# dotchen/LearningByCheating

Hardware: AMD Instinct MI355X
Metric: images/sec ImagePolicyModelSS phase-1 train @ bs256 (higher is better)
Workload: dtype bf16; 1 GPU; ImagePolicyModelSS(resnet34) phase-1 step vs BirdViewPolicyModelSS(resnet18) teacher [phase1_bs256_bf16], 160x384 RGB + 7x192x192 bird-view uint8 NHWC frames as the dataset stores them (2048-frame dataset per rank resident in HBM, a different batch every step), global batch 256 (256/GPU), bf16 MFMA operands and bf16 activation storage + f32 accumulate/master weights/gradients/BN/loss/Adam, local B; global_batch=256, parallelism=dp1

## Files before the change

### learningbycheating_amd/csrc/engine.cpp

```cpp
#include "engine.hpp"

#include <algorithm>
#include <stdlib.h>
#include <string.h>

namespace lbc {

namespace {
constexpr float kBnMomentum = 0.1f;
constexpr float kBnEps = 1e-5f;
size_t up64(size_t n) { return (n + 63) / 64 * 64; }
#define LBC_TRY(expr)            \
    do {                         \
        int rc__ = (expr);       \
        if (rc__) return rc__;   \
    } while (0)
}

int Net::add_tensor(const std::string& name, int kind, std::initializer_list<int> shape)
{
    TensorInfo ti;
    ti.name = name;
    ti.kind = kind;
    ti.ndim = (int)shape.size();
// ... 339 lines not shown
    if (!fn) { sync_fn_ = nullptr; sync_ctx_ = nullptr; sync_world_ = 1; sync_buf_ = nullptr; return LBC_OK; }
    LBC_REQUIRE(world >= 1 && buf && buf_floats >= kSyncFloats, "net.set_sync_bn: world_size >= 1 and a buffer of >= %d floats",
                kSyncFloats);
    sync_fn_ = fn; sync_ctx_ = ctx; sync_world_ = world; sync_buf_ = buf;
    return LBC_OK;
}

int Net::sync_rows(const float*& part, int& rows, int width, int n_local, hipStream_t s, float* local_lo, float* local_hi)
{
    if (!sync_fn_) return LBC_OK;
    LBC_REQUIRE(width + 1 <= kSyncFloats, "net: %d sums do not fit the SyncBN buffer", width);
    if (rows > kLbcFinalizeRows) {
        LBC_TRY(lbc_partial_reduce(part, rows, width, W(partial2_), 64, s));
        part = W(partial2_); rows = 64;
    }
    LBC_TRY(lbc_partial_reduce(part, rows, width, sync_buf_, 1, s, local_lo, local_hi, (float)n_local));
    if (sync_fn_(sync_ctx_, sync_buf_, width + 1, s) != 0) {
        lbc_set_error("net: the SyncBN all-reduce callback failed");
        return LBC_ELAUNCH;
    }
    part = sync_buf_; rows = 1;
    return LBC_OK;
}

int Net::bn_finalize(const BN& bn, int rows, long long count, int n_local, int train, hipStream_t s, bool update_running, const float* synced)
{
    const float* part = W(partial_);
    const float* nsum = nullptr;
    if (train && synced) {
        part = synced; rows = 1; nsum = synced + 2 * bn.C;
    } else if (train && sync_fn_) {
        LBC_TRY(sync_rows(part, rows, 2 * bn.C, n_local, s));
        nsum = part + 2 * bn.C;
    } else if (train && rows > kLbcFinalizeRows) {
        LBC_TRY(lbc_partial_reduce(W(partial_), rows, 2 * bn.C, W(partial2_), 64, s));
        part = W(partial2_);
        rows = 64;
    }
    BnFinalizeArgs f = fin_args(bn, part, rows, count, update_running);
    f.nsum = nsum; f.n_local = n_local; f.train = train;
    if (!train) { f.running_mean = P(bn.rm); f.running_var = P(bn.rv); f.num_batches_tracked = nullptr; }
    return lbc_bn_finalize(f, s);
}

BnFinalizeArgs Net::fin_args(const BN& bn, const float* part, int rows, long long count, bool update_running) const
{
    BnFinalizeArgs f;
    memset(&f, 0, sizeof(f));
    f.partial = part; f.rows = rows; f.C = bn.C; f.count = count;
    f.gamma = P(bn.g); f.beta = P(bn.b);
    f.running_mean = update_running ? P(bn.rm) : nullptr;
    f.running_var = update_running ? P(bn.rv) : nullptr;
    f.num_batches_tracked = update_running ? static_cast<long long*>(t_[bn.nbt].ptr) : nullptr;
    f.momentum = kBnMomentum; f.eps = kBnEps; f.train = 1;
    f.scale = W(bn.scale); f.shift = W(bn.shift); f.save_mean = W(bn.mean); f.save_invstd = W(bn.invstd);
    return f;
}

int Net::forward(int N, int train, const void* image, int image_u8, const float* velocity, const float* command, float* pred_sel,
                 float* pred_all, hipStream_t s)
{
    LBC_REQUIRE(N >= 1 && N <= d_.max_batch, "net.forward: batch %d outside [1,%d]", N, d_.max_batch);
    LBC_REQUIRE(image && velocity && command && pred_all, "net.forward: null argument");
    LBC_TRY(check_bound(false));
    lastN_ = N; last_train_ = train; ++generation_;
    const int H0 = d_.H, W0 = d_.W, Cin = d_.in_channels;
    const bool tr = train != 0;
    int rows = 0;

    LBC_TRY(lbc_copy_f32(command, W(cmd_), 4 * N, s));
    NormConst nc;
    memset(&nc, 0, sizeof(nc));
    nc.enabled = d_.normalize;
    const float m3[3] = {0.485f, 0.456f, 0.406f}, s3[3] = {0.229f, 0.224f, 0.225f};
    for (int i = 0; i < 3; ++i) { nc.mean[i] = m3[i]; nc.stdv[i] = s3[i]; }
    if (image_u8) LBC_TRY(lbc_prep_input_u8(static_cast<const unsigned char*>(image), W(xp_), bf16_, N, Cin, H0, W0, nc, s));
    else          LBC_TRY(lbc_prep_input(static_cast<const float*>(image), W(xp_), bf16_, N, Cin, H0, W0, nc, s));
    const bool reuse = frozen_ && derived_valid_ && !tr;
    if (act_bf16_ && !reuse) LBC_TRY(weight_prep(s));
    if (!tr && !reuse) LBC_TRY(bn_eval_prep(s));
    derived_valid_ = frozen_ && !tr;

    StemArgs st;
    st.xp = W(xp_); st.xp_bf16 = bf16_; st.w = P(stem_w_); st.y = W(y0_); st.stats = tr ? W(partial_) : nullptr;
    st.N = N; st.H = H0; st.W = W0; st.Cin = Cin; st.act_bf16 = act_bf16_; st.bf16 = bf16_;
    LBC_TRY(lbc_stem_fwd(st, s));
    if (tr) LBC_TRY(bn_finalize(stem_bn_, lbc_stem_rows(st), (long long)N * (H0 / 2) * (W0 / 2), N, train, s));
    PoolFwdArgs pf;
    pf.y = W(y0_); pf.scale = W(stem_bn_.scale); pf.shift = W(stem_bn_.shift); pf.p = W(p0_);
    pf.idx = reinterpret_cast<unsigned char*>(W(idx_));
    pf.N = N; pf.H = H0 / 2; pf.W = W0 / 2; pf.C = 64; pf.act_bf16 = act_bf16_;
    LBC_TRY(lbc_bn_relu_maxpool_fwd(pf, s));

    const float* x = W(p0_);
    for (Block& b : blocks_) {
        const long long pix = (long long)N * b.c1.OH * b.c1.OW;
        if (!tr) {
            LBC_TRY(conv_fwd(b.c1, x, N, false, &rows, s, nullptr, &b.b1, nullptr, true));
            const float* identity = x;
            if (b.has_ds) {
                LBC_TRY(conv_fwd(b.ds, x, N, false, &rows, s, nullptr, &b.bd, nullptr, false));
                identity = W(b.ds.y);
            }
            LBC_TRY(conv_fwd(b.c2, W(b.c1.y), N, false, &rows, s, nullptr, &b.b2, identity, true, W(b.out)));
            x = W(b.out);
            continue;
        }
        LBC_TRY(conv_fwd(b.c1, x, N, tr, &rows, s));
        const bool fold1 = !b.fuse_z1 && can_fold(rows, b.b1.C);
        if (!fold1) LBC_TRY(bn_finalize(b.b1, rows, pix, N, train, s));
        BnApplyArgs ap;
        if (b.fuse_z1) {
            LBC_TRY(conv_fwd(b.c2, W(b.c1.y), N, tr, &rows, s, &b.b1));
        } else {
            memset(&ap, 0, sizeof(ap));
            ap.x = W(b.c1.y); ap.y = W(b.z1); ap.pixels = pix; ap.C = b.c1.Cout;
            ap.scale = W(b.b1.scale); ap.shift = W(b.b1.shift); ap.relu = 1; ap.act_bf16 = act_bf16_;
            if (fold1) { ap.fold = 1; ap.fin = fin_args(b.b1, W(partial_), rows, pix); }
            LBC_TRY(lbc_bn_apply(ap, s));
            LBC_TRY(conv_fwd(b.c2, W(b.z1), N, tr, &rows, s));
        }
        const bool fold2 = can_fold(rows, b.b2.C) && (!b.has_ds || (size_t)lbc_cdiv(pix, 64) * 2 * b.bd.C <= partial2_floats_);
        const int rows2 = rows;
        if (!fold2) LBC_TRY(bn_finalize(b.b2, rows, pix, N, train, s));
        memset(&ap, 0, sizeof(ap));
        ap.x = W(b.c2.y); ap.y = W(b.out); ap.pixels = pix; ap.C = b.c2.Cout;
        ap.scale = W(b.b2.scale); ap.shift = W(b.b2.shift); ap.relu = 1; ap.act_bf16 = act_bf16_;
        if (fold2) { ap.fold = 1; ap.fin = fin_args(b.b2, W(partial_), rows2, pix); }
        if (b.has_ds) {
            float* dsp = fold2 ? W(partial2_) : W(partial_);
            LBC_TRY(conv_fwd(b.ds, x, N, tr, &rows, s, nullptr, nullptr, nullptr, false, nullptr, dsp, fold2 ? partial2_floats_ : partial_floats_));
            if (fold2 && can_fold(rows, b.bd.C)) { ap.rfold = 1; ap.rfin = fin_args(b.bd, dsp, rows, pix); }
            else if (fold2) LBC_TRY(lbc_bn_finalize(fin_args(b.bd, dsp, rows, pix), s));
            else LBC_TRY(bn_finalize(b.bd, rows, pix, N, train, s));
            ap.resid = W(b.ds.y); ap.rscale = W(b.bd.scale); ap.rshift = W(b.bd.shift);
        } else {
            ap.resid = x;
        }
        LBC_TRY(lbc_bn_apply(ap, s));
        x = W(b.out);
    }

    const Block& last = blocks_.back();
    const int th = last.c2.OH, tw = last.c2.OW;
    LBC_TRY(lbc_concat_velocity(x, velocity, W(hcat_), N, th * tw, 512, 128, act_bf16_, s));
    if (tr) {
        ChanReduceArgs cr;
        memset(&cr, 0, sizeof(cr));
        cr.x = W(hcat_); cr.partial = W(partial_); cr.pixels = (long long)N * th * tw; cr.C = 640; cr.act_bf16 = act_bf16_;
        cr.max_rows = fold_rows_for(cr.pixels, 640);
        LBC_TRY(lbc_chan_reduce(cr, 0, s));
        rows = lbc_chan_reduce_rows(cr.pixels, 640, cr.max_rows);
    }
    int pend_rows = rows;
    long long pend_count = (long long)N * th * tw;
    const float* din = W(hcat_);
    for (int i = 0; i < 3; ++i) {
        Deconv& D = dec_[i];
        IgemmArgs a;
        memset(&a, 0, sizeof(a));
        a.x = din; a.w = P(D.w); a.y = W(D.u); a.bias = P(D.bias); a.relu = 1;
        a.pre_scale = W(D.bn.scale); a.pre_shift = W(D.bn.shift);
        a.N = N; a.H = D.H; a.W = D.W; a.C = D.Cin;
        a.OH = 2 * D.H; a.OW = 2 * D.W; a.K = D.Cout;
        a.KH = 3; a.KW = 3; a.S = 2; a.P = 1;
        a.LH = D.H; a.LW = D.W; a.ostep = 2;
        a.M = N * D.H * D.W;
        a.stats = tr ? W(partial_) : nullptr;
        a.act_bf16 = act_bf16_;
        int wmajor = 0;
        if (act_bf16_) {
            a.w = W(D.wt); a.w_bf16 = 1; a.bf16 = 1; wmajor = 1;
        } else if (bf16_) {
            LBC_TRY(lbc_weight_transpose(P(D.w), W(wt_), D.Cin, 9, D.Cout, s));
            a.w = W(wt_); a.bf16 = 1; wmajor = 1;
// ... 624 lines not shown
```

### learningbycheating_amd/csrc/lbc_common.hpp

```cpp
#pragma once
#include <hip/hip_runtime.h>
#include <stddef.h>
#include <stdint.h>

typedef float f32x4 __attribute__((ext_vector_type(4)));
typedef float f32x16 __attribute__((ext_vector_type(16)));

#define LBC_OK 0
#define LBC_EINVAL (-1)
#define LBC_ELAUNCH (-2)
#define LBC_ESTATE (-3)

void lbc_set_error(const char* fmt, ...);
int lbc_check_launch(const char* what);

#define LBC_REQUIRE(cond, ...)                 \
    do {                                       \
        if (!(cond)) {                         \
            lbc_set_error(__VA_ARGS__);        \
            return LBC_EINVAL;                 \
        }                                      \
    } while (0)

static inline int lbc_cdiv(long long a, long long b) { return (int)((a + b - 1) / b); }

enum LbcOpt {
    kOptForceCfg = 0,
    kOptHaloBlocks,
    kOptHeadNoMfma,
    kOptNoSideStream,
    kOptNoGemm256,
    kOptGemm256MinTiles,
    kOptGemm256Cfg,
    kOptNoBnBwdFuse,
    kOptNoHdma,
    kOptHdmaCfg,
    kOptNoGldsPhased,
    kOptHdmaPersistWgs,
    kOptWgradTr2MinWgs,
    kOptNoC64pPre,
    kOptNoBnFold,
    kOptC64pBm,
    kOptHdmapSplit,
    kOptHdmaSmallBelow,
    kOptCount
};
long long lbc_opt(LbcOpt o);
static inline bool lbc_opt_on(LbcOpt o) { return lbc_opt(o) == 1; }

bool lbc_prof_on();
void lbc_prof_begin(const char* name, double flops, double bytes, hipStream_t s);
void lbc_prof_end(hipStream_t s);
void lbc_prof_note(const char* name, double bytes);
struct LbcProfScope {
    hipStream_t s; bool on;
    LbcProfScope(const char* name, double flops, double bytes, hipStream_t st) : s(st), on(lbc_prof_on()) {
        if (on) lbc_prof_begin(name, flops, bytes, s);
    }
    ~LbcProfScope() { if (on) lbc_prof_end(s); }
};

struct IgemmArgs {
    const void* x;
    const void* w;
    void* y;
    const float* post_scale;
    const float* post_shift;
    const float* bias;
    const void* resid;
    float* stats;
    const float* pre_scale;
    const float* pre_shift;
    int pre_relu;
    int N, H, W, C;
    int OH, OW, K;
    int KH, KW, S, P;
    int M;
    int LH, LW;
    int oy0, ox0, ostep;
    int nphase;
    int relu;
    int stat_row0;
    int bf16;
    int act_bf16;
    int w_bf16;
    const void* bnb_y;
    const float* bnb_scale;
    const float* bnb_shift;
    const float* bnb_mean;
    const float* bnb_invstd;
    const void* bnb_mask;
    float* split_ws;
    long long split_ws_floats;
};
bool lbc_igemm_fuses_bn_bwd(const IgemmArgs& a, int wmajor, int mode, int cfg);
bool lbc_igemm_fuses_bn_bwd_masked(const IgemmArgs& a, int wmajor, int mode, int cfg);

struct WeightPrepItem {
    const float* w;
    void* wn;
    void* wt;
    int A, T, B;
    int tile_begin;
};
static inline int lbc_weight_prep_tiles(int A, int T, int B) { return lbc_cdiv(A, 64) * lbc_cdiv(B, 64) * T; }
struct WeightPrepArgs {
    static const int kMax = 48;
    WeightPrepItem item[kMax];
    int count;
    int tiles;
};
int lbc_weight_prep(const WeightPrepArgs& a, hipStream_t s);

int lbc_igemm_rows(const IgemmArgs& a, int cfg);
int lbc_igemm_pick(long long M, int K);
int lbc_igemm_pick_for(const IgemmArgs& a, int mode);
constexpr int kLbcCfgGlds = 3;
constexpr int kLbcGldsCfgs = 7;
constexpr int kLbcCfgHdma = kLbcCfgGlds + kLbcGldsCfgs;
constexpr int kLbcHdmaCfgs = 5;
int lbc_conv_hdma_pick(const IgemmArgs& a, int mode);
int lbc_conv_hdma_rows(const IgemmArgs& a, int cfg);
int lbc_conv_hdma_launch(const IgemmArgs& a, int mode, int cfg, hipStream_t s);
int lbc_conv_c64p_launch(const IgemmArgs& a, int mode, hipStream_t s);
int lbc_conv_c64p_rows(const IgemmArgs& a);
bool lbc_conv_hdmap_phased(const IgemmArgs& a, int mode);
bool lbc_conv_hdmap_eligible(const IgemmArgs& a, int mode, int cfg);
// ... 50 lines not shown
```

### learningbycheating_amd/csrc/lbc_kernels.hpp

```cpp
#pragma once
#include "lbc_common.hpp"

constexpr int kLbcFinalizeRows = 1024;
struct BnFinalizeArgs {
    const float* partial;
    int rows, C;
    long long count;
    const float* nsum; int n_local;
    const float* gamma;
    const float* beta;
    float* running_mean;
    float* running_var;
    long long* num_batches_tracked;
    float* more_running_mean[3]; float* more_running_var[3]; long long* more_num_batches_tracked[3];
    float momentum, eps;
    int train;
    float* scale;
    float* shift;
    float* save_mean;
    float* save_invstd;
};
struct BnEvalItem {
    const float* gamma; const float* beta; const float* running_mean; const float* running_var;
    float* scale; float* shift; float* mean; float* invstd;
// ... 2 lines not shown
struct BnEvalArgs {
    static const int kMax = 48;
    BnEvalItem item[kMax];
    int count;
    float eps;
};
int lbc_bn_eval_prep(const BnEvalArgs& a, hipStream_t s);
int lbc_partial_reduce(const float* in, int rows, int cols, float* out, int out_rows, hipStream_t s, float* copy_lo = nullptr,
                       float* copy_hi = nullptr, float tail = -1.f);
int lbc_bn_finalize(const BnFinalizeArgs& a, hipStream_t s);

struct BnApplyArgs {
    const void* x; void* y;
    long long pixels; int C;
    const float* scale; const float* shift;
    const void* resid;
    const float* rscale;
    const float* rshift;
    int relu;
    int act_bf16;
    int fold, rfold;
    BnFinalizeArgs fin, rfin;
};
int lbc_bn_apply(const BnApplyArgs& a, hipStream_t s);
bool lbc_bn_fold_ok(int rows, int C);
int lbc_bn_fold_max_rows(int C);

struct ChanReduceArgs {
    const void* x;
    const void* dz;
    const void* mask;
    const float* mask_scale;
    const float* mask_shift;
    void* g_out;
    const float* mean;
    const float* invstd;
    float* partial;
    long long pixels; int C;
    long long pix_per_block;
    int act_bf16;
    int max_rows;
};
int lbc_chan_reduce_rows(long long pixels, int C, int max_rows = 0);
int lbc_chan_reduce(ChanReduceArgs a, int op, hipStream_t s);

struct BnBwdFinalizeArgs {
    const float* partial; int rows, C; long long count;
    const float* nsum; int n_local;
    const float* gamma; const float* mean; const float* invstd;
    int train;
    float* dgamma; float* dbeta;
    float* coefA; float* coefB; float* coefD;
};
int lbc_bn_bwd_finalize(const BnBwdFinalizeArgs& a, hipStream_t s);

struct BnBwdApplyArgs {
    const void* g; const void* mask; const void* x;
    const float* coefA; const float* coefB; const float* coefD;
    const float* mean; const float* invstd;
    void* dx;
    long long pixels; int C, Cout;
    int accum;
    int act_bf16;
    int fold;
    BnBwdFinalizeArgs fin;
};
int lbc_bn_bwd_apply(const BnBwdApplyArgs& a, hipStream_t s);

int lbc_copy_f32(const float* src, float* dst, long long n, hipStream_t s);
int lbc_concat_velocity(const void* t, const float* vel, void* h, int N, int hw, int Ct, int Cv, int act_bf16, hipStream_t s);

struct NormConst { float mean[8]; float stdv[8]; int enabled; };
int lbc_prep_input(const float* img_nchw, void* xp, int xp_bf16, int N, int C, int H, int W, const NormConst& nc, hipStream_t s);
int lbc_prep_input_u8(const unsigned char* img_nhwc, void* xp, int xp_bf16, int N, int C, int H, int W, const NormConst& nc, hipStream_t s);
struct StemArgs {
    const void* xp;
    int xp_bf16;
    const float* w;
    void* y;
    float* stats;
    int N, H, W, Cin;
    int act_bf16;
    int bf16;
};
int lbc_stem_rows(const StemArgs& a);
int lbc_stem_fwd(const StemArgs& a, hipStream_t s);
struct StemWgradArgs {
    const void* xp; int xp_bf16; const void* dy; float* partial;
    int N, H, W, Cin, nsplit;
    int act_bf16;
    int bf16;
    const void* bn_y;
    const float* bn_coefA; const float* bn_coefB; const float* bn_coefD; const float* bn_mean; const float* bn_invstd;
};
bool lbc_stem_wgrad_fuses_bn_bwd(int Cin, int bf16);
int lbc_stem_wgrad_split(int N, int H, int W, int Cin, int bf16);
int lbc_stem_wgrad(const StemWgradArgs& a, hipStream_t s);

struct PoolFwdArgs {
    const void* y;
    const float* scale; const float* shift;
    void* p;
    unsigned char* idx;
    int N, H, W, C;
    int act_bf16;
};
int lbc_bn_relu_maxpool_fwd(const PoolFwdArgs& a, hipStream_t s);
struct PoolBwdArgs {
    const void* dp;
    const unsigned char* idx;
    const void* y;
    const float* scale; const float* shift;
    const float* mean; const float* invstd;
    void* g;
    float* partial;
    int N, H, W, C;
    long long pix_per_block;
    int act_bf16;
};
int lbc_pool_bwd_rows(int N, int H, int W, int C);
int lbc_maxpool_relu_bwd_reduce(PoolBwdArgs a, hipStream_t s);

struct HeadArgs {
    const void* h;
    int act_bf16;
    const float* mean[4];
    const float* invstd[4];
    const float* gamma[4];
    const float* beta[4];
    const float* w[4];
    const float* bias[4];
    const float* cmd;
    const float* pos_x[4];
    const float* pos_y[4];
    float* pred_all;
    float* pred_sel;
    float* rowstat;
    int N, OH, OW;
    float* scratch;
    int nslice;
    int wsplit;
};
int lbc_head_fwd(const HeadArgs& a, hipStream_t s);
struct HeadBwdArgs {
    HeadArgs f;
    const float* d_all;
    const float* d_sel;
    float* s_partial;
    void* dh;
    const float* chan_coef;
};
int lbc_head_bwd_rows(const HeadArgs& f);
int lbc_head_bwd_max_rows(int max_batch);
int lbc_head_bwd_reduce(const HeadBwdArgs& a, hipStream_t s);
struct HeadBwdFinalizeArgs {
    const float* s_partial; int rows; long long count;
    const float* nsum; int n_local;
    const float* gamma[4]; const float* beta[4]; const float* w[4];
    const float* mean; const float* invstd;
    float* dgamma[4]; float* dbeta[4]; float* dw[4]; float* dbias[4];
    float* chan_coef;
    int coef_only;
};
int lbc_head_bwd_finalize(const HeadBwdFinalizeArgs& a, hipStream_t s);
int lbc_head_bwd_apply(const HeadBwdArgs& a, hipStream_t s);

enum { kAugBlur = 0, kAugNoise = 1, kAugCoarseDropout = 2, kAugDropout = 3, kAugAdd = 4, kAugMultiply = 5, kAugContrast = 6 };
struct WarpParams {
    double im[6];
// ... 35 lines not shown
```

### learningbycheating_amd/csrc/lbc_util.cpp

```cpp
#include "lbc_common.hpp"
#include <stdarg.h>
#include <stdio.h>

static thread_local char g_err[512] = "";

void lbc_set_error(const char* fmt, ...)
{
    va_list ap;
    va_start(ap, fmt);
    vsnprintf(g_err, sizeof(g_err), fmt, ap);
    va_end(ap);
}

int lbc_check_launch(const char* what)
{
    hipError_t e = hipGetLastError();
    if (e != hipSuccess) {
        lbc_set_error("%s: launch failed: %s", what, hipGetErrorString(e));
        return LBC_ELAUNCH;
    }
    return LBC_OK;
}

extern "C" const char* lbc_last_error(void) { return g_err; }

#include <stdlib.h>
#include <mutex>
extern "C" char** environ;
#include <string.h>
namespace {
const char* const kOptNames[kOptCount] = {
    "LBC_FORCE_CFG", "LBC_HALO_BLOCKS", "LBC_HEAD_NO_MFMA", "LBC_NO_SIDE_STREAM", "LBC_NO_GEMM256", "LBC_GEMM256_MIN_TILES", "LBC_GEMM256_CFG",
    "LBC_NO_BN_BWD_FUSE", "LBC_NO_HDMA", "LBC_HDMA_CFG", "LBC_NO_GLDS_PHASED", "LBC_HDMA_PERSIST_WGS", "LBC_WGRAD_TR2_MIN_WGS", "LBC_NO_C64P_PRE",
    "LBC_NO_BN_FOLD", "LBC_C64P_BM", "LBC_HDMAP_SPLIT", "LBC_HDMA_SMALL_BELOW"};
struct OptTable {
    long long v[kOptCount];
    OptTable()
    {
        for (int i = 0; i < kOptCount; ++i) {
            const char* e = getenv(kOptNames[i]);
            v[i] = (e && *e) ? atoll(e) : -1;
        }
        for (char** ep = environ; ep && *ep; ++ep) {
            if (strncmp(*ep, "LBC_", 4)) continue;
            const char* eq = strchr(*ep, '=');
            const size_t n = eq ? (size_t)(eq - *ep) : strlen(*ep);
            bool known = (n == 17 && !strncmp(*ep, "LBC_PROF_LAUNCHES", n)) || (n == 15 && !strncmp(*ep, "LBC_PIN_STAGING", n)) || !strncmp(*ep, "LBC_ARCH", 8) || !strncmp(*ep, "LBC_BUILD_", 10) || !strncmp(*ep, "LBC_TEST_", 9) || !strncmp(*ep, "LBC_EMU_", 8);
            for (int i = 0; i < kOptCount && !known; ++i) known = strlen(kOptNames[i]) == n && !strncmp(*ep, kOptNames[i], n);
            if (!known) fprintf(stderr, "liblbc_hip: environment variable %.*s is not an option of this library (ignored); see include/lbc_hip.h, lbc_config_set\n", (int)n, *ep);
        }
    }
};
OptTable& opts() { static OptTable t; return t; }
}
long long lbc_opt(LbcOpt o) { return opts().v[o]; }
extern "C" int lbc_config_set(const char* name, long long value)
{
    LBC_REQUIRE(name, "config_set: null name");
    for (int i = 0; i < kOptCount; ++i)
        if (!strcmp(name, kOptNames[i])) { opts().v[i] = value; return LBC_OK; }
    lbc_set_error("config_set: unknown option %s", name);
    return LBC_EINVAL;
}
extern "C" long long lbc_config_get(const char* name)
{
    if (name)
        for (int i = 0; i < kOptCount; ++i)
            if (!strcmp(name, kOptNames[i])) return opts().v[i];
    return -1;
}

int lbc_zero_page(const void** p)
{
    static void* pages[64] = {nullptr};
    static std::mutex mu;
    int dev = 0;
    if (hipGetDevice(&dev) != hipSuccess || dev < 0 || dev >= 64) { lbc_set_error("zero_page: bad device"); return LBC_ELAUNCH; }
    std::lock_guard<std::mutex> lock(mu);
    if (!pages[dev]) {
        void* q = nullptr;
        if (hipMalloc(&q, 256) != hipSuccess || hipMemset(q, 0, 256) != hipSuccess) { lbc_set_error("zero_page: allocation failed"); return LBC_ELAUNCH; }
        pages[dev] = q;
    }
    *p = pages[dev];
    return LBC_OK;
}

#include <map>
#include <string>
#include <vector>
namespace {
struct ProfRec { const char* name; double flops, bytes; hipEvent_t e0, e1; };
bool g_prof = false;
std::vector<ProfRec> g_recs;
}
bool lbc_prof_on() { return g_prof; }
void lbc_prof_begin(const char* name, double flops, double bytes, hipStream_t s)
{
    ProfRec r;
    r.name = name; r.flops = flops; r.bytes = bytes;
    (void)hipEventCreate(&r.e0); (void)hipEventCreate(&r.e1);
    (void)hipEventRecord(r.e0, s);
    g_recs.push_back(r);
}
void lbc_prof_end(hipStream_t s) { if (!g_recs.empty()) (void)hipEventRecord(g_recs.back().e1, s); }
void lbc_prof_note(const char* name, double bytes)
{
    ProfRec r;
    r.name = name; r.flops = 0.0; r.bytes = bytes; r.e0 = nullptr; r.e1 = nullptr;
    if (g_recs.empty()) g_recs.push_back(r); else g_recs.insert(g_recs.end() - 1, r);
}

extern "C" int lbc_profile_enable(int on)
{
    g_prof = on != 0;
    return 0;
}
// ... 31 lines not shown
```

### learningbycheating_amd/csrc/stem.hip

```cpp
#include "lbc_common.hpp"
#include "lbc_act.hpp"
#include "lbc_kernels.hpp"
#include <type_traits>

namespace {

template <typename XT>
__global__ __launch_bounds__(256) void prep_input_k(const float* __restrict__ img, XT* __restrict__ xp, int N, int C,
                                                    int H, int W, NormConst nc)
{
    const int Hp = H + 6, Wp = W + 6;
    const long long total = (long long)N * Hp * Wp;
    const long long stride = (long long)gridDim.x * blockDim.x;
    for (long long i = (long long)blockIdx.x * blockDim.x + threadIdx.x; i < total; i += stride) {
        const int xq = (int)(i % Wp);
        const long long t = i / Wp;
        const int yq = (int)(t % Hp);
        const int n = (int)(t / Hp);
        const int x = xq - 3, y = yq - 3;
        const bool in = (unsigned)x < (unsigned)W && (unsigned)y < (unsigned)H;
        XT* dst = xp + (size_t)i * C;
        for (int c = 0; c < C; ++c) {
            float v = 0.f;
            if (in) {
// ... 625 lines not shown
        for (int q = 0; q < NLD; ++q)
            if (br[q] < 7) *reinterpret_cast<unsigned*>(&sBand[buf][br[q] * RS + bj[q] * 4]) = regs[q];
    };

    float s1 = 0.f, s2 = 0.f;
    int tile, tend, it = 0;
    {
        const int nwg = gridDim.x, b = blockIdx.x;
        const int xcd = b & 7, q = nwg >> 3, rr = nwg & 7;
        const int logical = (xcd < rr ? xcd * (q + 1) : rr * (q + 1) + (xcd - rr) * q) + (b >> 3);
        const int per = (ntiles + nwg - 1) / nwg;
        tile = logical * per;
        tend = tile + per < ntiles ? tile + per : ntiles;
    }
    if (tile < tend) band_load(tile);
    __syncthreads();
    if (tile < tend) band_store(0);
    __syncthreads();
    for (; tile < tend; ++tile, ++it) {
        const int buf = it & 1;
        const int next = tile + 1 < tend ? tile + 1 : ntiles;
        if (next < ntiles) band_load(next);
        const int xt = tile % tiles_x;
        const int t2 = tile / tiles_x;
        const int oy = t2 % OH, n = t2 / OH;
        const int ox0 = xt * BX;
        f32x16 acc;
#pragma unroll
        for (int e = 0; e < 16; ++e) acc[e] = 0.f;
        const char* band = &sBand[buf][0] + ((32 * wm + l31) * 2 * CIN + 8 * kh) * 2;
#pragma unroll
        for (int r = 0; r < 7; ++r)
#pragma unroll
            for (int g = 0; g < KG; ++g) {
                const unsigned* src = reinterpret_cast<const unsigned*>(band + r * RS + g * 32);
                typedef unsigned u32x4 __attribute__((ext_vector_type(4)));
                const u32x4 raw = {src[0], src[1], src[2], src[3]};
                acc = __builtin_amdgcn_mfma_f32_32x32x16_bf16(__builtin_bit_cast(bf16x8, raw), bw[r][g], acc, 0, 0, 0);
            }
        const int col = 32 * wn + l31;
#pragma unroll
        for (int e = 0; e < 16; ++e) {
            const int prow = 32 * wm + (e & 3) + 8 * (e >> 2) + 4 * kh;
            const float v = acc[e];
            Act<T>::st1(&sOut[prow * OLD + col], v);
            if (ox0 + prow < OW) { s1 += v; s2 += v * v; }
        }
        if (next < ntiles) band_store(buf ^ 1);
        __syncthreads();
        {
            constexpr int EPT = 16;
            const int prow = tid >> 2, c0 = (tid & 3) * EPT;
            if (ox0 + prow < OW) {
                T* dst = static_cast<T*>(a.y) + ((size_t)(n * OH + oy) * OW + (size_t)(ox0 + prow)) * 64 + c0;
                const T* srcp = &sOut[prow * OLD + c0];
#pragma unroll
                for (int v = 0; v < EPT * (int)sizeof(T) / 16; ++v)
                    reinterpret_cast<f32x4*>(dst)[v] = reinterpret_cast<const f32x4*>(srcp)[v];
            }
        }
        __syncthreads();
    }
    if (a.stats) {
        s1 += __shfl_xor(s1, 32);
        s2 += __shfl_xor(s2, 32);
        if (kh == 0) { sRed[wm][0][32 * wn + l31] = s1; sRed[wm][1][32 * wn + l31] = s2; }
        __syncthreads();
        if (tid < 64) {
            float* dst = a.stats + (size_t)blockIdx.x * 2 * 64;
            dst[tid] = sRed[0][0][tid] + sRed[1][0][tid];
            dst[64 + tid] = sRed[0][1][tid] + sRed[1][1][tid];
        }
    }
}

static int stem_rows_grid(int N, int H, int W, int Cin)
{
    const long long tiles = (long long)N * (H / 2) * lbc_cdiv(W / 2, 64);
    const long long grid = 256 * (Cin == 3 ? 3 : 2);
    return (int)(tiles < grid ? tiles : grid);
}
static bool stem_fwd_rows(const StemArgs& a) { return a.bf16 != 0; }

}

int lbc_prep_input_u8(const unsigned char* img_nhwc, void* xp, int xp_bf16, int N, int C, int H, int W, const NormConst& nc, hipStream_t s)
{
    LBC_REQUIRE(C <= 8, "prep_input: at most 8 channels");
    const long long total = (long long)N * (H + 6) * (W + 6);
    long long blocks = (total + 255) / 256;
    if (blocks > 4096) blocks = 4096;
    LbcProfScope prof("prep_input", 0.0, 1.0 * N * H * (double)W * C + (xp_bf16 ? 2.0 : 4.0) * (double)total * C, s);
    const bool small = total + blocks * 256 < (1ll << 31);
#define LBC_PU(XT, CINv)                                                                                                                 \
    do {                                                                                                                                 \
        if (small) hipLaunchKernelGGL((prep_input_u8_k<XT, CINv, unsigned>), dim3((unsigned)blocks), dim3(256), 0, s, img_nhwc, static_cast<XT*>(xp), N, C, H, W, nc);  \
        else       hipLaunchKernelGGL((prep_input_u8_k<XT, CINv, long long>), dim3((unsigned)blocks), dim3(256), 0, s, img_nhwc, static_cast<XT*>(xp), N, C, H, W, nc); \
    } while (0)
#define LBC_PUC(XT)                                                                                                                      \
    do {                                                                                                                                 \
        if (C == 3) LBC_PU(XT, 3);                                                                                                       \
        else if (C == 7) LBC_PU(XT, 7);                                                                                                  \
        else LBC_PU(XT, 0);                                                                                                              \
    } while (0)
    if (xp_bf16) LBC_PUC(__bf16);
    else         LBC_PUC(float);
#undef LBC_PUC
#undef LBC_PU
    return lbc_check_launch("prep_input_u8");
}

int lbc_prep_input(const float* img_nchw, void* xp, int xp_bf16, int N, int C, int H, int W, const NormConst& nc, hipStream_t s)
{
    LBC_REQUIRE(C <= 8, "prep_input: at most 8 channels");
    const long long total = (long long)N * (H + 6) * (W + 6);
    long long blocks = (total + 255) / 256;
    if (blocks > 4096) blocks = 4096;
    LbcProfScope prof("prep_input", 0.0, 4.0 * N * H * (double)W * C + (xp_bf16 ? 2.0 : 4.0) * (double)total * C, s);
    if (xp_bf16) hipLaunchKernelGGL(prep_input_k<__bf16>, dim3((unsigned)blocks), dim3(256), 0, s, img_nchw, static_cast<__bf16*>(xp), N, C, H, W, nc);
    else         hipLaunchKernelGGL(prep_input_k<float>, dim3((unsigned)blocks), dim3(256), 0, s, img_nchw, static_cast<float*>(xp), N, C, H, W, nc);
    return lbc_check_launch("prep_input");
}

int lbc_stem_rows(const StemArgs& a)
{
    if (stem_fwd_rows(a)) return stem_rows_grid(a.N, a.H, a.W, a.Cin);
    return lbc_cdiv((long long)a.N * (a.H / 2) * (a.W / 2), 128);
}

int lbc_stem_fwd(const StemArgs& a, hipStream_t s)
{
    LBC_REQUIRE(a.Cin == 3 || a.Cin == 7, "stem: Cin=%d unsupported (3 or 7)", a.Cin);
    LBC_REQUIRE(a.H % 2 == 0 && a.W % 2 == 0, "stem: odd image size");
    LBC_REQUIRE((long long)a.N * (a.H + 6) * (a.W + 6) * a.Cin < (1ll << 31), "stem: input too large");
    const dim3 grid((unsigned)lbc_stem_rows(a));
    const double Ms = (double)a.N * (a.H / 2) * (a.W / 2);
    LbcProfScope prof("stem_fwd", 2.0 * Ms * 64 * 49 * a.Cin, (a.xp_bf16 ? 2.0 : 4.0) * (double)a.N * (a.H + 6) * (a.W + 6) * a.Cin + (a.act_bf16 ? 2.0 : 4.0) * Ms * 64, s);
    LBC_REQUIRE(!a.act_bf16 || a.bf16, "stem: bf16 output needs bf16 = 1");
    if (stem_fwd_rows(a)) {
        LBC_REQUIRE(a.xp_bf16, "stem: the bf16 kernels read a bf16 padded image");
        const int tx = lbc_cdiv(a.W / 2, 64);
        const int ntiles = a.N * (a.H / 2) * tx;
#define LBC_K(T, CI) hipLaunchKernelGGL((stem_fwd_rows_k<CI, T>), grid, dim3(256), 0, s, a, ntiles, tx)
        if (a.Cin == 3) LBC_DISPATCH_ACT(a.act_bf16, LBC_K, 3);
        else            LBC_DISPATCH_ACT(a.act_bf16, LBC_K, 7);
#undef LBC_K
        return lbc_check_launch("stem_fwd");
    }
    if (a.Cin == 3) hipLaunchKernelGGL((stem_fwd_k<3, float>), grid, dim3(256), 0, s, a);
    else            hipLaunchKernelGGL((stem_fwd_k<7, float>), grid, dim3(256), 0, s, a);
    return lbc_check_launch("stem_fwd");
}

static bool stem_wgrad_rows(int Cin, int bf16) { return bf16 && Cin == 3; }
bool lbc_stem_wgrad_fuses_bn_bwd(int Cin, int bf16) { return stem_wgrad_rows(Cin, bf16) && !lbc_opt_on(kOptNoBnBwdFuse); }

int lbc_stem_wgrad_split(int N, int H, int W, int Cin, int bf16)
{
    if (stem_wgrad_rows(Cin, bf16)) {
        const long long chunks = ((long long)N * (H / 2) * (W / 2) + 63) / 64;
        long long ng = chunks / 8;
        if (ng > 512) ng = 512;
        if (ng < 1) ng = 1;
        return (int)(2 * ng);
    }
    const long long chunks = ((long long)N * (H / 2) * (W / 2) + 31) / 32;
// ... 42 lines not shown
```

Baseline: 18150 images/sec.

## Fuse eval-mode stem conv with BN, ReLU and maxpool into one kernel

Adds a kernel that computes the 7x7 stride-2 stem convolution with MFMA, then applies the 3x3/2 maxpool and the folded BN scale/shift plus ReLU in the same pass. It uses the sign of gamma so the max can be taken before the affine step. It is used only in eval-mode forward, i.e. the frozen teacher, and removes the full-resolution stem activation round trip through HBM and the separate pool kernel. In exchange it adds a complex row-band pipeline with overlap recompute across work-unit boundaries and shared-memory carry state.

```diff
diff --git a/learningbycheating_amd/csrc/engine.cpp b/learningbycheating_amd/csrc/engine.cpp
--- a/learningbycheating_amd/csrc/engine.cpp
+++ b/learningbycheating_amd/csrc/engine.cpp
@@ -445,15 +445,21 @@
     derived_valid_ = frozen_ && !tr;
 
     StemArgs st;
+    memset(&st, 0, sizeof(st));
     st.xp = W(xp_); st.xp_bf16 = bf16_; st.w = P(stem_w_); st.y = W(y0_); st.stats = tr ? W(partial_) : nullptr;
     st.N = N; st.H = H0; st.W = W0; st.Cin = Cin; st.act_bf16 = act_bf16_; st.bf16 = bf16_;
-    LBC_TRY(lbc_stem_fwd(st, s));
-    if (tr) LBC_TRY(bn_finalize(stem_bn_, lbc_stem_rows(st), (long long)N * (H0 / 2) * (W0 / 2), N, train, s));
-    PoolFwdArgs pf;
-    pf.y = W(y0_); pf.scale = W(stem_bn_.scale); pf.shift = W(stem_bn_.shift); pf.p = W(p0_);
-    pf.idx = reinterpret_cast<unsigned char*>(W(idx_));
-    pf.N = N; pf.H = H0 / 2; pf.W = W0 / 2; pf.C = 64; pf.act_bf16 = act_bf16_;
-    LBC_TRY(lbc_bn_relu_maxpool_fwd(pf, s));
+    if (!tr && lbc_stem_pool_ok(H0, W0, Cin, act_bf16_, bf16_)) {
+        st.y = nullptr; st.gamma = P(stem_bn_.g); st.scale = W(stem_bn_.scale); st.shift = W(stem_bn_.shift); st.p = W(p0_);
+        LBC_TRY(lbc_stem_pool_fwd(st, s));
+    } else {
+        LBC_TRY(lbc_stem_fwd(st, s));
+        if (tr) LBC_TRY(bn_finalize(stem_bn_, lbc_stem_rows(st), (long long)N * (H0 / 2) * (W0 / 2), N, train, s));
+        PoolFwdArgs pf;
+        pf.y = W(y0_); pf.scale = W(stem_bn_.scale); pf.shift = W(stem_bn_.shift); pf.p = W(p0_);
+        pf.idx = reinterpret_cast<unsigned char*>(W(idx_));
+        pf.N = N; pf.H = H0 / 2; pf.W = W0 / 2; pf.C = 64; pf.act_bf16 = act_bf16_;
+        LBC_TRY(lbc_bn_relu_maxpool_fwd(pf, s));
+    }
 
     const float* x = W(p0_);
     for (Block& b : blocks_) {
diff --git a/learningbycheating_amd/csrc/lbc_common.hpp b/learningbycheating_amd/csrc/lbc_common.hpp
--- a/learningbycheating_amd/csrc/lbc_common.hpp
+++ b/learningbycheating_amd/csrc/lbc_common.hpp
@@ -43,6 +43,7 @@
     kOptC64pBm,
     kOptHdmapSplit,
     kOptHdmaSmallBelow,
+    kOptNoStemPoolFuse,
     kOptCount
 };
 long long lbc_opt(LbcOpt o);
diff --git a/learningbycheating_amd/csrc/lbc_kernels.hpp b/learningbycheating_amd/csrc/lbc_kernels.hpp
--- a/learningbycheating_amd/csrc/lbc_kernels.hpp
+++ b/learningbycheating_amd/csrc/lbc_kernels.hpp
@@ -108,9 +108,14 @@
     int N, H, W, Cin;
     int act_bf16;
     int bf16;
+    const float* gamma;
+    const float* scale; const float* shift;
+    void* p;
 };
 int lbc_stem_rows(const StemArgs& a);
 int lbc_stem_fwd(const StemArgs& a, hipStream_t s);
+bool lbc_stem_pool_ok(int H, int W, int Cin, int act_bf16, int bf16);
+int lbc_stem_pool_fwd(const StemArgs& a, hipStream_t s);
 struct StemWgradArgs {
     const void* xp; int xp_bf16; const void* dy; float* partial;
     int N, H, W, Cin, nsplit;
diff --git a/learningbycheating_amd/csrc/lbc_util.cpp b/learningbycheating_amd/csrc/lbc_util.cpp
--- a/learningbycheating_amd/csrc/lbc_util.cpp
+++ b/learningbycheating_amd/csrc/lbc_util.cpp
@@ -32,7 +32,8 @@
 const char* const kOptNames[kOptCount] = {
     "LBC_FORCE_CFG", "LBC_HALO_BLOCKS", "LBC_HEAD_NO_MFMA", "LBC_NO_SIDE_STREAM", "LBC_NO_GEMM256", "LBC_GEMM256_MIN_TILES", "LBC_GEMM256_CFG",
     "LBC_NO_BN_BWD_FUSE", "LBC_NO_HDMA", "LBC_HDMA_CFG", "LBC_NO_GLDS_PHASED", "LBC_HDMA_PERSIST_WGS", "LBC_WGRAD_TR2_MIN_WGS", "LBC_NO_C64P_PRE",
-    "LBC_NO_BN_FOLD", "LBC_C64P_BM", "LBC_HDMAP_SPLIT", "LBC_HDMA_SMALL_BELOW"};
+    "LBC_NO_BN_FOLD", "LBC_C64P_BM", "LBC_HDMAP_SPLIT", "LBC_HDMA_SMALL_BELOW",
+    "LBC_NO_STEM_POOL_FUSE"};
 struct OptTable {
     long long v[kOptCount];
     OptTable()
diff --git a/learningbycheating_amd/csrc/stem.hip b/learningbycheating_amd/csrc/stem.hip
--- a/learningbycheating_amd/csrc/stem.hip
+++ b/learningbycheating_amd/csrc/stem.hip
@@ -731,6 +731,200 @@
 }
 static bool stem_fwd_rows(const StemArgs& a) { return a.bf16 != 0; }
 
+constexpr int kStemPoolMaxOW = 192;
+template <int CIN>
+__global__ __launch_bounds__(256, 2) void stem_pool_rows_k(StemArgs a, int nunits)
+{
+    using T = __bf16;
+    constexpr int L = 7 * CIN;
+    constexpr int KG = (L + 15) / 16;
+    constexpr int BX = 32;
+    constexpr int BL = (2 * (BX - 1) + 7) * CIN;
+    constexpr int BD = (BL + 1) / 2;
+    constexpr int RS = ((2 * (BX - 1) * CIN + KG * 16) * 2 + 15) / 16 * 16;
+    constexpr int BR = 9;
+    constexpr int NLD = (BR * BD + 255) / 256;
+    constexpr int OLD = 64 + 8;
+    __shared__ __attribute__((aligned(16))) char sBand[2][BR * RS];
+    __shared__ __attribute__((aligned(16))) T sOut[2][2 * BX * OLD];
+    __shared__ __attribute__((aligned(8))) T sCv[kStemPoolMaxOW / 2 * 64];
+
+    const __bf16* xpad = static_cast<const __bf16*>(a.xp);
+    const int tid = threadIdx.x, lane = tid & 63, wave = tid >> 6;
+    const int l31 = lane & 31, kh = lane >> 5;
+    const int wm = wave & 1, wn = wave >> 1;
+    const int OH = a.H / 2, OW = a.W / 2, PH = OH / 2, PW = OW / 2;
+    const int nsub = OW / BX;
+    const int Hp = a.H + 6, Wp = a.W + 6;
+    const long long total_elems = (long long)a.N * Hp * Wp * CIN;
+
+    for (int i = tid; i < 2 * BR * RS / 4; i += 256) reinterpret_cast<unsigned*>(&sBand[0][0])[i] = 0u;
+
+    bf16x8 bw[7][KG];
+    {
+        const float* wrow = a.w + (size_t)(32 * wn + l31) * (49 * CIN);
+#pragma unroll
+        for (int r = 0; r < 7; ++r)
+#pragma unroll
+            for (int g = 0; g < KG; ++g)
+#pragma unroll
+                for (int i = 0; i < 8; ++i) {
+                    const int k = 16 * g + 8 * kh + i;
+                    bw[r][g][i] = (__bf16)(k < L ? wrow[r * L + (k < L ? k : 0)] : 0.f);
+                }
+    }
+    const int pw = tid >> 4, pc = (tid & 15) * 4;
+    float kmul[4], psc[4], psh[4];
+#pragma unroll
+    for (int e = 0; e < 4; ++e) {
+        const float g = a.gamma[pc + e];
+        kmul[e] = g > 0.f ? 1.f : (g < 0.f ? -1.f : 0.f);
+        psc[e] = a.scale[pc + e];
+        psh[e] = a.shift[pc + e];
+    }
+
+    int br[NLD], bj[NLD];
+#pragma unroll
+    for (int q = 0; q < NLD; ++q) {
+        const int idx = tid + 256 * q;
+        br[q] = idx / BD;
+        bj[q] = idx - br[q] * BD;
+    }
+    unsigned regs[NLD];
+    auto band_load = [&](int item) {
+        const int j = item % nsub, u = item / nsub;
+        const int oy = u % PH, n = u / PH;
+        const long long e0 = ((long long)(n * Hp + 4 * oy) * Wp + 2 * BX * j) * CIN;
+#pragma unroll
+        for (int q = 0; q < NLD; ++q) {
+            const long long e = e0 + (long long)br[q] * Wp * CIN + 2 * bj[q];
+            const bool ok = br[q] < BR && e + 1 < total_elems;
+            regs[q] = ok ? *reinterpret_cast<const unsigned*>(xpad + e) : 0u;
+        }
+    };
+    auto band_store = [&](int buf) {
+#pragma unroll
+        for (int q = 0; q < NLD; ++q)
+            if (br[q] < BR) *reinterpret_cast<unsigned*>(&sBand[buf][br[q] * RS + bj[q] * 4]) = regs[q];
+    };
+
+    int item, iend, it = 0, first_out;
+    {
+        const int nwg = gridDim.x, b = blockIdx.x;
+        const int xcd = b & 7, q = nwg >> 3, rr = nwg & 7;
+        const int logical = (xcd < rr ? xcd * (q + 1) : rr * (q + 1) + (xcd - rr) * q) + (b >> 3);
+        const int per = (nunits + nwg - 1) / nwg;
+        const int u0 = logical * per;
+        const int u1 = u0 + per < nunits ? u0 + per : nunits;
+        first_out = u0 * nsub;
+        item = (u0 < u1 && u0 % PH != 0 ? u0 - 1 : u0) * nsub;
+        iend = u0 < u1 ? u1 * nsub : item;
+    }
+    if (item < iend) band_load(item);
+    __syncthreads();
+    if (item < iend) band_store(0);
+    __syncthreads();
+    for (; item < iend; ++item, ++it) {
+        const int buf = it & 1;
+        const int next = item + 1 < iend ? item + 1 : -1;
+        if (next >= 0) band_load(next);
+        const int j = item % nsub, u = item / nsub;
+        const int oy = u % PH, n = u / PH;
+        const bool live = item >= first_out;
+        f32x16 acc;
+#pragma unroll
+        for (int e = 0; e < 16; ++e) acc[e] = 0.f;
+        const char* band = &sBand[buf][0] + 2 * wm * RS + (l31 * 2 * CIN + 8 * kh) * 2;
+#pragma unroll
+        for (int r = 0; r < 7; ++r)
+#pragma unroll
+            for (int g = 0; g < KG; ++g) {
+                const unsigned* src = reinterpret_cast<const unsigned*>(band + r * RS + g * 32);
+                typedef unsigned u32x4 __attribute__((ext_vector_type(4)));
+                const u32x4 raw = {src[0], src[1], src[2], src[3]};
+                acc = __builtin_amdgcn_mfma_f32_32x32x16_bf16(__builtin_bit_cast(bf16x8, raw), bw[r][g], acc, 0, 0, 0);
+            }
+        T* so = sOut[buf];
+        const T* sp = sOut[buf ^ 1];
+        const int col = 32 * wn + l31;
+#pragma unroll
+        for (int e = 0; e < 16; ++e) {
+            const int prow = 32 * wm + (e & 3) + 8 * (e >> 2) + 4 * kh;
+            const float v = acc[e];
+            Act<T>::st1(&so[prow * OLD + col], v);
+        }
+        if (next >= 0) band_store(buf ^ 1);
+        __syncthreads();
+        {
+            const int ox = (BX / 2) * j + pw;
+            float hv[2][4];
+#pragma unroll
+            for (int rr = 0; rr < 2; ++rr) {
+                const bool ok0 = pw > 0 || j > 0;
+                const T* p0 = pw > 0 ? &so[(32 * rr + 2 * pw - 1) * OLD + pc] : &sp[(32 * rr + 31) * OLD + pc];
+                const bf16x4 t0 = *reinterpret_cast<const bf16x4*>(ok0 ? p0 : &so[(32 * rr) * OLD + pc]);
+                const bf16x4 t1 = *reinterpret_cast<const bf16x4*>(&so[(32 * rr + 2 * pw) * OLD + pc]);
+                const bf16x4 t2 = *reinterpret_cast<const bf16x4*>(&so[(32 * rr + 2 * pw + 1) * OLD + pc]);
+#pragma unroll
+                for (int e = 0; e < 4; ++e) {
+                    float bv = ok0 ? (float)t0[e] : (float)t1[e];
+                    const float v1 = (float)t1[e], v2 = (float)t2[e];
+                    if (v1 * kmul[e] > bv * kmul[e]) bv = v1;
+                    if (v2 * kmul[e] > bv * kmul[e]) bv = v2;
+                    hv[rr][e] = bv;
+                }
+            }
+            if (live) {
+                const bool top = oy > 0;
+                const bf16x4 cv = *reinterpret_cast<const bf16x4*>(&sCv[ox * 64 + pc]);
+                f32x4 best;
+#pragma unroll
+                for (int e = 0; e < 4; ++e) {
+                    float bv = top ? (float)cv[e] : hv[0][e];
+                    if (hv[0][e] * kmul[e] > bv * kmul[e]) bv = hv[0][e];
+                    if (hv[1][e] * kmul[e] > bv * kmul[e]) bv = hv[1][e];
+                    best[e] = fmaxf(bv * psc[e] + psh[e], 0.f);
+                }
+                const size_t o = ((size_t)(n * PH + oy) * PW + (size_t)ox) * 64 + pc;
+                *reinterpret_cast<bf16x4*>(static_cast<T*>(a.p) + o) = __builtin_convertvector(best, bf16x4);
+            }
+            bf16x4 nv;
+#pragma unroll
+            for (int e = 0; e < 4; ++e) nv[e] = (__bf16)hv[1][e];
+            *reinterpret_cast<bf16x4*>(&sCv[ox * 64 + pc]) = nv;
+        }
+        __syncthreads();
+    }
+}
+
+static int stem_pool_grid(int N, int H, int Cin)
+{
+    const long long units = (long long)N * (H / 4);
+    long long grid = 256 * (Cin == 3 ? 3 : 2);
+    if (lbc_opt(kOptHaloBlocks) > 0 && lbc_opt(kOptHaloBlocks) < grid) grid = lbc_opt(kOptHaloBlocks);
+    return (int)(units < grid ? units : grid);
+}
+
+}
+
+bool lbc_stem_pool_ok(int H, int W, int Cin, int act_bf16, int bf16)
+{
+    return act_bf16 && bf16 && (Cin == 3 || Cin == 7) && H % 4 == 0 && W % 64 == 0 && W / 2 <= kStemPoolMaxOW && !lbc_opt_on(kOptNoStemPoolFuse);
+}
+
+int lbc_stem_pool_fwd(const StemArgs& a, hipStream_t s)
+{
+    LBC_REQUIRE(a.act_bf16 && a.bf16 && a.xp_bf16 && (a.Cin == 3 || a.Cin == 7) && a.H % 4 == 0 && a.W % 64 == 0 && a.W / 2 <= kStemPoolMaxOW,
+                "stem_pool: unsupported shape / mode (lbc_stem_pool_ok)");
+    LBC_REQUIRE((long long)a.N * (a.H + 6) * (a.W + 6) * a.Cin < (1ll << 31), "stem_pool: input too large");
+    LBC_REQUIRE(a.gamma && a.scale && a.shift && a.p, "stem_pool: null argument");
+    const int units = a.N * (a.H / 4);
+    const dim3 grid((unsigned)stem_pool_grid(a.N, a.H, a.Cin));
+    const double Ms = (double)a.N * (a.H / 2) * (a.W / 2), Mp = Ms / 4;
+    LbcProfScope prof("stem_pool_fwd", 2.0 * Ms * 64 * 49 * a.Cin, 2.0 * (double)a.N * (a.H + 6) * (a.W + 6) * a.Cin + 2.0 * Mp * 64, s);
+    if (a.Cin == 3) hipLaunchKernelGGL((stem_pool_rows_k<3>), grid, dim3(256), 0, s, a, units);
+    else            hipLaunchKernelGGL((stem_pool_rows_k<7>), grid, dim3(256), 0, s, a, units);
+    return lbc_check_launch("stem_pool_fwd");
 }
 
 int lbc_prep_input_u8(const unsigned char* img_nhwc, void* xp, int xp_bf16, int N, int C, int H, int W, const NormConst& nc, hipStream_t s)
```

Result: no change. 18310 images/sec (median of 6 runs) (+0.9%).
